# johannah/drqv2

Hardware: AMD Instinct MI355X
Metric: agent updates/sec (batch=256, 9x84x84 obs) (higher is better)
Workload: dtype f32; 1 GPU; cheetah_run batch_size=256/GPU (256 global) 9x84x84 u8 obs, A=6, feature_dim=50, hidden_dim=1024, fp32, use_tb=True; parallelism=dp1, global_batch=256

## Files before the change

drqv2_amd/_lib.py:

```python
import ctypes as C
import os

HERE = os.path.dirname(os.path.abspath(__file__))
LIB_PATH = os.path.join(HERE, "libdrqv2_hip.so")

c_float_p = C.c_void_p
c_u8_p = C.c_void_p
stream_t = C.c_void_p


class DrqStep(C.Structure):
    _fields_ = [
        ("B", C.c_int), ("global_B", C.c_int), ("C", C.c_int), ("A", C.c_int), ("F", C.c_int), ("H", C.c_int),
        ("obs", c_u8_p), ("next_obs", c_u8_p),
        ("action", c_float_p), ("reward", c_float_p), ("discount", c_float_p),
        ("shift_obs", c_float_p), ("shift_next", c_float_p),
        ("noise_critic", c_float_p), ("noise_actor", c_float_p),
        ("base_grid", c_float_p),
        ("params", c_float_p), ("grads", c_float_p), ("adam_m", c_float_p), ("adam_v", c_float_p),
        ("ws", c_float_p), ("ws_bytes", C.c_size_t),
        ("sums", c_float_p),
        ("lr", C.c_double), ("tau", C.c_double),
        ("std", C.c_float), ("clip", C.c_float),
        ("step_critic", C.c_long), ("step_enc", C.c_long), ("step_actor", C.c_long),
# ... 77 lines not shown
    "drq_tanh_bwd": (I, [P, P, P, L, P]),
    "drq_param_layout": (I, [I, I, I, I, C.POINTER(L), I]),
    "drq_step_ws_bytes": (SZ, [I, I, I, I, I]),
    "drq_step_ws_offset": (L, [I, I, I, I, I, I]),
    "drq_update_phase": (I, [C.POINTER(DrqStep), I]),
    "drq_update_phase_bc": (I, [C.POINTER(DrqStep), I, F]),
    "drq_update_phase_per": (I, [C.POINTER(DrqStep), I, P, P]),
    "drq_act_forward": (I, [C.POINTER(DrqStep), P, I, P]),
    "drq_act_ws_bytes": (SZ, [I, I, I, I, I]),
    "drq_act_batch": (I, [P, I, I, I, I, P, I, P, F, P, P, P, SZ, P]),
    "drq_publish_sums": (I, [P, P, C.c_uint, P]),
    "drq_rng_draws": (I, [C.c_uint64, C.c_uint64, I, I, I, P, P, P, P, P]),
}

WS_IDS = ["AUG", "ACT1", "ACT2", "ACT3", "FEAT", "Z_NEXT", "Z_OBS", "HA_T", "HA_C", "H_AN", "H_AO", "Q", "TQ",
          "DQ", "MU_O", "DY4", "DY3", "DY2", "DY1", "DZ_C", "DZ_A", "HA_C2", "P1", "P2", "C1", "C2"]

PHASE_ALL, PHASE_CRITIC, PHASE_ACTOR, PHASE_OPT = -1, 0, 1, 2
PHASE_ENCODE, PHASE_CRITIC_HEADS, PHASE_CONV_BACKWARD, PHASE_ACTOR_FORWARD, PHASE_ACTOR_BACKWARD = 3, 4, 5, 6, 7
PHASE_ENCODER_OPT, PHASE_ACTOR_OPT = 8, 9
PHASE_CRITIC_OPT, PHASE_ACTOR_LOSS, PHASE_POLYAK, PHASE_REDRAW = 10, 11, 12, 13

_lib = None


class DrqError(RuntimeError):
    pass


def load():
    global _lib
# ... 41 lines not shown
```

drqv2_amd/csrc/conv1aug.hip:

```cpp
#include "common.h"
#include "internal.h"
#include "wino_u.h"

namespace {

constexpr int H = 84, C = 9, PAD = 4, S = 92, HW = H * H;
constexpr int HO = 41, PO = HO * HO;
constexpr int NBAND = 5;
constexpr int MAXR = 9;
constexpr int NROWS = 2 * MAXR + 1;
constexpr int SROWS = NROWS + 2;
constexpr int XPL = 42;
constexpr int XPITCH = 2 * XPL;
constexpr int HQ = H / 4;
constexpr int CP = 5, NS = CP * 9;
constexpr int XS_FLOATS = C * NROWS * XPITCH;
constexpr int U8_DWORDS = C * SROWS * HQ;
constexpr int NDMA = (U8_DWORDS + 63) / 64;
constexpr int U8_ALLOC = NDMA * 64;
constexpr int NTHR = 256;
constexpr int NWAVE = NTHR / 64;
constexpr int MAXU = 64;
constexpr int LDS_BYTES = (XS_FLOATS + U8_ALLOC + H + 3 * MAXU) * 4;

struct Conv1AugArgs {
  const uint8_t* obs[2];
  const long* fidx[2];
  const float* shift[2];
  const float* base;
  const float* w;
  const float* bias;
  float* xaug;
  float* y;
  int n, n_store;
  unsigned y_bytes;
  int stagger;
  const float* wino_w[3];
  float* wino_u;
  int n_rider;
};

typedef float f32x2 __attribute__((ext_vector_type(2)));
typedef __bf16 bf16x8_c1 __attribute__((ext_vector_type(8)));
typedef unsigned u32x4_c1 __attribute__((ext_vector_type(4)));
typedef unsigned u32x2_c1 __attribute__((ext_vector_type(2)));

__device__ __forceinline__ unsigned pack_bf16_c1(float lo, float hi) {
  typedef __bf16 bf16x2_c1 __attribute__((ext_vector_type(2)));
  const bf16x2_c1 v = {(__bf16)lo, (__bf16)hi};
  return __builtin_bit_cast(unsigned, v);
}

__device__ __forceinline__ float div255(float v) {
  const float r = 1.0f / 255.0f;
// ... 263 lines not shown
      }
      }
      const int oy = done.r0 + oyl;
      if constexpr (YN) {
        const int yo = p0 < npix ? (((done.f * HO + oy) * HO + ox) * 16 + half * 2) * 4 : (int)0x80000000u;
#pragma unroll
        for (int g4 = 0; g4 < 4; ++g4) {
          float v[4];
#pragma unroll
          for (int e = 0; e < 4; ++e) v[e] = acc[4 * g4 + e] > 0.f ? acc[4 * g4 + e] : 0.f;
          const u32x2_c1 o = {pack_bf16_c1(v[0], v[1]), pack_bf16_c1(v[2], v[3])};
          __builtin_amdgcn_raw_buffer_store_b64(o, yrsrc, yo, g4 * 16, 0);
        }
        continue;
      }
      const int yoff = p0 < npix ? (((done.f * 32 + 4 * half) * HO + oy) * HO + ox) * 4 : (int)0x80000000u;
#pragma unroll
      for (int r = 0; r < 16; ++r) {
        const float v = acc[r] > 0.f ? acc[r] : 0.f;
        __builtin_amdgcn_raw_buffer_store_b32(__float_as_uint(v), yrsrc, yoff, ((r & 3) + 8 * (r >> 2)) * PO * 4, 0);
      }
    }
  }
}

}

int drq_conv1_aug_fwd_any(int bf_mma, const uint8_t* obs, const float* shift, const uint8_t* obs1, const float* shift1,
                          const float* base_grid, const float* w, const float* bias, float* xaug, float* y, int n,
                          int n_store, hipStream_t st, const float* const* wino_w, float* wino_u, const long* fidx0,
                          const long* fidx1) {
  if (!obs || !shift || !obs1 || !shift1 || !base_grid || !w || !bias || !y || n <= 0 || n_store < 0 || n_store > 2 * n)
    return DRQ_EARG;
  if (n_store > 0 && !xaug) return DRQ_EARG;
  if (((uintptr_t)obs & 3) || ((uintptr_t)obs1 & 3)) return DRQ_EARG;
  const size_t yb = (size_t)2 * n * 32 * PO * (bf_mma == 2 ? 2 : 4);
  if (yb >= (1ull << 31) || (bf_mma == 2 && ((uintptr_t)y & 15))) return DRQ_EARG;
  Conv1AugArgs a{};
  a.obs[0] = obs; a.obs[1] = obs1;
  a.fidx[0] = fidx0; a.fidx[1] = fidx1;
  a.shift[0] = shift; a.shift[1] = shift1;
  a.base = base_grid; a.w = w; a.bias = bias; a.xaug = xaug; a.y = y;
  a.n = n; a.n_store = n_store; a.y_bytes = (unsigned)yb; a.stagger = 1;
  if (wino_w && wino_u) {
    for (int l = 0; l < 3; ++l) a.wino_w[l] = wino_w[l];
    a.wino_u = wino_u;
    a.n_rider = 6;
  }
  static bool attr_set_dev[kMaxDevices] = {};
  bool& attr_set = attr_set_dev[drq_device()];
  if (!attr_set) {
    hipError_t e = hipFuncSetAttribute((const void*)conv1_aug_kernel<false>, hipFuncAttributeMaxDynamicSharedMemorySize,
                                       LDS_BYTES);
    if (e == hipSuccess)
      e = hipFuncSetAttribute((const void*)conv1_aug_kernel<true>, hipFuncAttributeMaxDynamicSharedMemorySize, LDS_BYTES);
    if (e == hipSuccess)
      e = hipFuncSetAttribute((const void*)conv1_aug_kernel<true, true>, hipFuncAttributeMaxDynamicSharedMemorySize,
// ... 46 lines not shown
```

drqv2_amd/csrc/conv_wino.hip:

```cpp
#include "common.h"
#include "internal.h"
#include "wino_u.h"
#include <type_traits>

namespace {

struct WinoArgs {
  const float* x;
  const float* w;
  const float* pre;
  const float* bias;
  const float* mask;
  float* y;
  int y_bs, y_cs, y_rs, y_off;
  unsigned x_bytes, y_bytes, mask_bytes;
  int nb;
  int relu;
  int wmode;
  int stagger;
};

typedef unsigned u32x4w __attribute__((ext_vector_type(4)));
typedef unsigned u32x2w __attribute__((ext_vector_type(2)));
typedef float f32x2w __attribute__((ext_vector_type(2)));

constexpr int kStagger = 0;

template <int HIN, bool MASK, bool RELU>
__global__ __launch_bounds__(256, 2) void conv3x3_wino_kernel(WinoArgs a) {
#pragma clang fp contract(off)
  constexpr int HOUT = HIN - 2;
  constexpr int TH = (HOUT + 1) / 2;
  constexpr int TT = TH * TH;
  constexpr int PLANE = HIN * HIN * 4;
  __shared__ __attribute__((aligned(16))) float U[16 * 8 * 64 * 2];

  const int tid = threadIdx.x;
  const int lane = tid & 63;
  const int wid = tid >> 6;
  const int tl = lane & 15;
  const int kk = lane >> 4;

  if (a.pre) {
    const f32x4* src = reinterpret_cast<const f32x4*>(a.pre);
    f32x4* dst = reinterpret_cast<f32x4*>(U);
// ... 10 lines not shown
  for (int h = 0; h < 2; ++h)
#pragma unroll
    for (int r = 0; r < 4; ++r) bv[h][r] = a.bias ? a.bias[16 * h + 4 * kk + r] : 0.f;
  __syncthreads();

  if (a.stagger) {
    const unsigned hwid = __builtin_amdgcn_s_getreg((4 << 0) | (0 << 6) | (31 << 11));
    if (hwid & 1u)
      for (int q = 0; q < a.stagger; ++q) __builtin_amdgcn_s_sleep(16);
  }

  const __amdgpu_buffer_rsrc_t xrs = __builtin_amdgcn_make_buffer_rsrc((void*)a.x, 0, a.x_bytes, 0x00020000);
  const __amdgpu_buffer_rsrc_t yrs = __builtin_amdgcn_make_buffer_rsrc((void*)a.y, 0, a.y_bytes, 0x00020000);
  const __amdgpu_buffer_rsrc_t mrs =
      __builtin_amdgcn_make_buffer_rsrc((void*)a.mask, 0, a.mask ? a.mask_bytes : 0, 0x00020000);
  constexpr int kDrop = (int)0x80000000u;

  const int ntile = a.nb * TT;
  const int nunit = (ntile + 15) >> 4;
  const int nwave = (int)gridDim.x * 4;
  const f32x2w* Ul = reinterpret_cast<const f32x2w*>(U) + lane;

  auto patch_voff = [&](int unit) {
    int t = unit * 16 + tl;
    t = t < ntile ? t : ntile - 1;
    const int b = t / TT, rem = t - b * TT;
    const int ty = rem / TH, tx = rem - ty * TH;
    return (((b * 32 + kk) * HIN + 2 * ty) * HIN + 2 * tx) * 4;
  };
  auto load_patch_row = [&](float (&d)[16], int voff, int c, int i) {
    const u32x4w v = __builtin_amdgcn_raw_buffer_load_b128(xrs, voff, c * (4 * PLANE) + i * (HIN * 4), 0);
// ... 49 lines not shown
    const int t = valid ? t0 : ntile - 1;
    const int b = t / TT, rem = t - b * TT;
    const int ty = rem / TH, tx = rem - ty * TH;
    const bool c1ok = 2 * tx + 1 < HOUT, r1ok = 2 * ty + 1 < HOUT;
    const int ybase = (a.y_off + b * a.y_bs + (4 * kk) * a.y_cs + (2 * ty) * a.y_rs + 2 * tx) * 4;
    const int mbase = (((b * 32 + 4 * kk) * HOUT + 2 * ty) * HOUT + 2 * tx) * 4;
    int o64[2], o32[2];
#pragma unroll
    for (int i = 0; i < 2; ++i) {
      const bool rowok = valid && (i == 0 || r1ok);
      o64[i] = (rowok && c1ok) ? ybase : kDrop;
      o32[i] = (rowok && !c1ok) ? ybase : kDrop;
    }
    f32x4 acc[16][2];
    u32x2w mk[2][4][2];
#pragma unroll
    for (int c = 0; c < 8; ++c) {
      asm volatile("" ::: "memory");
      float t[16];
#pragma unroll
      for (int j = 0; j < 4; ++j) {
        t[0 * 4 + j] = d[0 * 4 + j] - d[2 * 4 + j];
        t[1 * 4 + j] = d[1 * 4 + j] + d[2 * 4 + j];
        t[2 * 4 + j] = d[2 * 4 + j] - d[1 * 4 + j];
        t[3 * 4 + j] = d[1 * 4 + j] - d[3 * 4 + j];
      }
      __builtin_amdgcn_sched_barrier(0);
      load_A(A1, c, 1);
      __builtin_amdgcn_sched_barrier(0);
      float V[16];
// ... 17 lines not shown
          if (c == 0) {
            const f32x4 z = {0.f, 0.f, 0.f, 0.f};
            const f32x4 b0 = {bv[0][0], bv[0][1], bv[0][2], bv[0][3]}, b1 = {bv[1][0], bv[1][1], bv[1][2], bv[1][3]};
            if constexpr (HSEL != 1) acc[pos][0] = __builtin_amdgcn_mfma_f32_16x16x4f32(Ap[0], V[pos], pos == 5 ? b0 : z, 0, 0, 0);
            if constexpr (HSEL != 0) acc[pos][1] = __builtin_amdgcn_mfma_f32_16x16x4f32(Ap[1], V[pos], pos == 5 ? b1 : z, 0, 0, 0);
          } else {
            if constexpr (HSEL != 1) acc[pos][0] = __builtin_amdgcn_mfma_f32_16x16x4f32(Ap[0], V[pos], acc[pos][0], 0, 0, 0);
            if constexpr (HSEL != 0) acc[pos][1] = __builtin_amdgcn_mfma_f32_16x16x4f32(Ap[1], V[pos], acc[pos][1], 0, 0, 0);
          }
        }
      };
      half_step(A0, 0);
      __builtin_amdgcn_sched_barrier(0);
      load_A(A0, (c + 1) & 7, 0);
      if constexpr (MASK) {
        if (c == 7) {
          constexpr int h0 = HSEL == 1 ? 1 : 0;
#pragma unroll
          for (int r = 0; r < 4; ++r)
#pragma unroll
            for (int i = 0; i < 2; ++i)
              mk[h0][r][i] = __builtin_amdgcn_raw_buffer_load_b64(mrs, mbase + i * (HOUT * 4),
                                                                  (16 * h0 + r) * (HOUT * HOUT * 4), 0);
        }
      }
      __builtin_amdgcn_sched_barrier(0);
      half_step(A1, 1);
      __builtin_amdgcn_sched_barrier(0);
    }
    {
      if constexpr (MASK && HSEL == 2) {
#pragma unroll
        for (int r = 0; r < 4; ++r)
#pragma unroll
          for (int i = 0; i < 2; ++i)
            mk[1][r][i] = __builtin_amdgcn_raw_buffer_load_b64(mrs, mbase + i * (HOUT * 4), (16 + r) * (HOUT * HOUT * 4), 0);
        __builtin_amdgcn_sched_barrier(0);
      }
      const int ycs4 = a.y_cs * 4, yrs4 = a.y_rs * 4;
#pragma unroll
      for (int h = (HSEL == 1 ? 1 : 0); h < (HSEL == 0 ? 1 : 2); ++h)
#pragma unroll
        for (int r = 0; r < 4; ++r) {
          float s[2][4];
#pragma unroll
          for (int j = 0; j < 4; ++j) {
            const float m0 = acc[0 * 4 + j][h][r], m1 = acc[1 * 4 + j][h][r], m2 = acc[2 * 4 + j][h][r],
                        m3 = acc[3 * 4 + j][h][r];
            s[0][j] = (m0 + m1) + m2;
            s[1][j] = (m1 - m2) - m3;
          }
          const int co = (16 * h + r);
#pragma unroll
          for (int i = 0; i < 2; ++i) {
            float y0 = (s[i][0] + s[i][1]) + s[i][2];
            float y1 = (s[i][1] - s[i][2]) - s[i][3];
            if constexpr (RELU) {
              y0 = __builtin_fmaxf(y0, 0.f);
              y1 = __builtin_fmaxf(y1, 0.f);
            }
            if constexpr (MASK) {
              const unsigned q0 = mk[h][r][i][0], q1 = mk[h][r][i][1];
              y0 = __uint_as_float(q0) > 0.f ? y0 : 0.f;
              y1 = __uint_as_float(q1) > 0.f ? y1 : 0.f;
            }
            const int soff = co * ycs4 + i * yrs4;
            const u32x2w pk = {__float_as_uint(y0), __float_as_uint(y1)};
            __builtin_amdgcn_raw_buffer_store_b64(pk, yrs, o64[i], soff, 0);
            __builtin_amdgcn_raw_buffer_store_b32(__float_as_uint(y0), yrs, o32[i], soff, 0);
          }
        }
    }
    voff = nvoff;
  };
  for (int i = 0; i < nfull; ++i) body(std::integral_constant<int, 2>{}, item_unit(i), item_unit(i + 1 < nitem ? i + 1 : i));
  if (has_half) {
    if (half_h == 0) body(std::integral_constant<int, 0>{}, half_unit, half_unit);
    else body(std::integral_constant<int, 1>{}, half_unit, half_unit);
  }
}

template <int HIN>
int launch_wino(const WinoArgs& a0, hipStream_t st) {
  WinoArgs a = a0;
  a.stagger = kStagger;
  constexpr int HOUT = HIN - 2, TH = (HOUT + 1) / 2;
  const long nunit = ((long)a.nb * TH * TH + 15) / 16;
  long blocks = (nunit + 3) / 4;
  const long cap = 2L * drq_num_cus();
  if (blocks > cap) blocks = cap;
  if (blocks < 1) blocks = 1;
  const dim3 g((unsigned)blocks), t(256);
  if (a.mask && a.relu) hipLaunchKernelGGL((conv3x3_wino_kernel<HIN, true, true>), g, t, 0, st, a);
  else if (a.mask) hipLaunchKernelGGL((conv3x3_wino_kernel<HIN, true, false>), g, t, 0, st, a);
  else if (a.relu) hipLaunchKernelGGL((conv3x3_wino_kernel<HIN, false, true>), g, t, 0, st, a);
  else hipLaunchKernelGGL((conv3x3_wino_kernel<HIN, false, false>), g, t, 0, st, a);
  DRQ_LAUNCH_CHECK();
  return DRQ_OK;
}

}

int drq_conv3x3_fwd_wino_pre(const float* x, const float* w, const float* u_image, const float* bias, float* y, int nb,
                             int hin, int relu, long y_bs, long y_cs, long y_rs, long y_off, hipStream_t st) {
  if (!x || !w || !y || nb <= 0) return DRQ_EARG;
  const size_t xb = (size_t)nb * 32 * hin * hin * 4;
  const size_t yb = (size_t)nb * y_bs * 4;
  if (xb >= (1ull << 31) || yb >= (1ull << 31) || y_off < 0 || y_bs <= 0) return DRQ_EARG;
  WinoArgs a{x, w, u_image, bias, nullptr, y, (int)y_bs, (int)y_cs, (int)y_rs, (int)y_off, (unsigned)xb, (unsigned)yb, 0u, nb, relu, 0, 0};
  if (hin == 41) return launch_wino<41>(a, st);
  if (hin == 39) return launch_wino<39>(a, st);
  if (hin == 37) return launch_wino<37>(a, st);
  return DRQ_EARG;
}

int drq_conv3x3_dgrad_wino_pre(const float* dy_pad, const float* w, const float* u_image, const float* mask, float* dx,
                               int nb, int hout, long dx_bs, long dx_cs, long dx_rs, long dx_off, hipStream_t st) {
  if (!dy_pad || !w || !dx || nb <= 0) return DRQ_EARG;
  const int hp = hout + 4;
  const size_t xb = (size_t)nb * 32 * hp * hp * 4;
  const size_t yb = (size_t)nb * dx_bs * 4;
  const size_t mb = (size_t)nb * 32 * (hout + 2) * (hout + 2) * 4;
  if (xb >= (1ull << 31) || yb >= (1ull << 31) || dx_off < 0 || dx_bs <= 0) return DRQ_EARG;
  WinoArgs a{dy_pad, w, u_image, nullptr, mask, dx, (int)dx_bs, (int)dx_cs, (int)dx_rs, (int)dx_off, (unsigned)xb, (unsigned)yb,
             (unsigned)mb, nb, 0, 1, 0};
  if (hp == 39) return launch_wino<39>(a, st);
  if (hp == 41) return launch_wino<41>(a, st);
  if (hp == 43) return launch_wino<43>(a, st);
  return DRQ_EARG;
}

DRQ_API int drq_conv3x3_fwd_wino(const float* x, const float* w, const float* bias, float* y, int nb, int hin, int relu,
                                 long y_bs, long y_cs, long y_rs, long y_off, hipStream_t st) {
  return drq_conv3x3_fwd_wino_pre(x, w, nullptr, bias, y, nb, hin, relu, y_bs, y_cs, y_rs, y_off, st);
}

DRQ_API int drq_conv3x3_dgrad_wino(const float* dy_pad, const float* w, const float* mask, float* dx, int nb, int hout,
                                   long dx_bs, long dx_cs, long dx_rs, long dx_off, hipStream_t st) {
  return drq_conv3x3_dgrad_wino_pre(dy_pad, w, nullptr, mask, dx, nb, hout, dx_bs, dx_cs, dx_rs, dx_off, st);
}
```

drqv2_amd/csrc/internal.h:

```cpp
#pragma once
#include "common.h"

int drq_ln_tanh_fwd_multi_ex(int n, const float* const* z, int ldz, const float* const* gamma,
                             const float* const* beta, float* const* out, const int* ldo, float* const* xhat,
                             float* const* rstd, int rows, int F, const float* const* tail, const int* tail_ld,
                             int tail_n, hipStream_t st);
int drq_ln_tanh_fwd_multi_part(int n, const float* const* z, int ldz, const float* const* gamma,
                               const float* const* beta, float* const* out, const int* ldo, float* const* xhat,
                               float* const* rstd, int rows, int F, const float* const* tail, const int* tail_ld,
                               int tail_n, const float* part, const float* const* bias, int splitk, hipStream_t st);
int drq_ln_tanh_bwd_part(const float* dh0, int ld0, const float* dh1, int ld1, const float* h, int ldh,
                         const float* xhat, const float* rstd, const float* gamma, float* dz, float* dln,
                         float* dgamma, float* dbeta, int rows, int F, const float* part, int splitk, int nprob,
                         int ldp, hipStream_t st);
int drq_ln_param_grad(const float* dln, const float* xhat, float* dgamma, float* dbeta, int rows, int F,
                      hipStream_t st);
int drq_qout_bwd_td(const float* tq1, const float* tq2, const float* q1, const float* q2, const float* reward,
                    const float* discount, float inv_global_B, float* sums, const float* const* h,
                    const float* const* w, float* const* dh, float* const* dw, float* const* db, int B, int H,
                    hipStream_t st);
int drq_qout_bwd_td_w(const float* tq1, const float* tq2, const float* q1, const float* q2, const float* reward,
                      const float* discount, const float* is_weight, float inv_global_B, float* sums, float* td_abs,
                      const float* const* h, const float* const* w, float* const* dh, float* const* dw,
                      float* const* db, int B, int H, hipStream_t st);
// ... 52 lines not shown
                          long lddx, const float* const* mask, int ldmask, int Brows, int Nout, int Kin, hipStream_t st);

int drq_lnl1_fwd(int njobs, const float* const* part, const float* const* z, const float* const* bias,
                 const float* const* gamma, const float* const* beta, float* const* out, const int* ldo,
                 float* const* xhat, float* const* rstd, const float* const* tail, const int* tail_ld, const int* tail_n,
                 const int* rows, const int* nheads, const float* const* w, const float* const* b, float* const* y, int F,
                 int H, int splitk, long slab, hipStream_t st);
int drq_polout_l1_fwd(const float* p2, const float* w3, const float* b3, float* p3, int rows, int srow0, int H, int A,
                      int F, float std, float clip, int use_clip, const float* noise_hi, float* mu_hi, float* ha_hi,
                      long lda_hi, const float* noise_lo, float* mu_lo, float* ha_lo, long lda_lo, int nheads,
                      const float* const* w, const float* const* b, float* const* y, hipStream_t st);

int drq_conv1_aug_fwd_any(int bf_mma, const uint8_t* obs, const float* shift, const uint8_t* obs1, const float* shift1,
                          const float* base_grid, const float* w, const float* bias, float* xaug, float* y, int n,
                          int n_store, hipStream_t st, const float* const* wino_w, float* wino_u, const long* fidx0,
                          const long* fidx1);

int drq_conv3x3_fwd_wino_pre(const float* x, const float* w, const float* u_image, const float* bias, float* y, int nb,
                             int hin, int relu, long y_bs, long y_cs, long y_rs, long y_off, hipStream_t st);
int drq_conv3x3_dgrad_wino_pre(const float* dy_pad, const float* w, const float* u_image, const float* mask, float* dx,
                               int nb, int hout, long dx_bs, long dx_cs, long dx_rs, long dx_off, hipStream_t st);

int drq_conv3x3_fwd_bf16_lay(const void* x, const float* w, const float* bias, void* y, int nb, int hin, int relu,
                             long y_bs, long y_cs, long y_rs, long y_off, int lay, hipStream_t st);
int drq_conv3x3_dgrad_bf16_lay(const void* dy_pad, const float* w, const void* mask, void* dx, int nb, int hout,
                               long dx_bs, long dx_cs, long dx_rs, long dx_off, int lay, hipStream_t st);
int drq_conv3x3_wgrad_partial_bf16_lay(const void* x, const void* dy, int nb, int hin, long dy_bs, long dy_cs, long dy_rs,
                                       long dy_off, float* part, size_t part_bytes, int* nblocks, int lay,
                                       hipStream_t st);
int drq_conv3x3_wgrad_partial_bf16(const float* x, const float* dy, int nb, int hin, long dy_bs, long dy_cs, long dy_rs,
                                   long dy_off, float* part, size_t part_bytes, int* nblocks, hipStream_t st);

constexpr int kActMaxRows = 256;
struct ActWeights {
  const float *enc_w[4], *enc_b[4];
  const float *trunk_w, *trunk_b, *ln_g, *ln_b;
// ... 19 lines not shown
```

drqv2_amd/csrc/step.hip:

```cpp
#include "common.h"
#include "internal.h"
#include "../../include/drqv2_hip.h"

namespace {

constexpr long R = 32L * 35 * 35;
inline long al64(long x) { return (x + 63) & ~63L; }
inline long al512(long x) { return (x + 511) & ~511L; }

struct HeadOff {
  long trunk_w, trunk_b, ln_g, ln_b;
  long w[2][3], b[2][3];
};
enum { SEG_ENC, SEG_CRITIC, SEG_ACTOR, SEG_TARGET };
struct ParamLayout {
  long enc_w[4], enc_b[4];
  HeadOff critic, actor, target;
  long seg[8];
  long total;
  long flat[50];
  int nflat;
  long seg_beg(int net) const { return seg[2 * net]; }
  long seg_len(int net) const { return seg[2 * net + 1] - seg[2 * net]; }
};
// ... 47 lines not shown
}

struct WsLayout {
  long off[64];
  long total;
};
constexpr long kGemmWsFloats = 16L * 1024 * 1024;
enum {
  W_AUG = DRQ_WS_AUG, W_ACT1 = DRQ_WS_ACT1, W_ACT2 = DRQ_WS_ACT2, W_ACT3 = DRQ_WS_ACT3, W_FEAT = DRQ_WS_FEAT,
  W_Z_NEXT = DRQ_WS_Z_NEXT, W_Z_OBS = DRQ_WS_Z_OBS, W_HA_T = DRQ_WS_HA_T, W_HA_C = DRQ_WS_HA_C,
  W_H_AN = DRQ_WS_H_AN, W_H_AO = DRQ_WS_H_AO, W_Q = DRQ_WS_Q, W_TQ = DRQ_WS_TQ, W_DQ = DRQ_WS_DQ,
  W_MU_O = DRQ_WS_MU_O, W_DY4 = DRQ_WS_DY4, W_DY3 = DRQ_WS_DY3, W_DY2 = DRQ_WS_DY2, W_DY1 = DRQ_WS_DY1,
  W_DZ_C = DRQ_WS_DZ_C, W_DZ_A = DRQ_WS_DZ_A, W_HA_C2 = DRQ_WS_HA_C2,
  W_P1 = DRQ_WS_P1, W_P2 = DRQ_WS_P2,
  W_C1 = DRQ_WS_C1, W_C2 = DRQ_WS_C2,
  W_XHAT_C = DRQ_WS_NBUF_PUBLIC, W_RSTD_C, W_XHAT_A, W_RSTD_A, W_Z_C2,
  W_HROWS, W_P3, W_Z4,
  W_T1, W_T2,
  W_DC2, W_DC1, W_DHA, W_DLN, W_DPRE, W_DP2, W_DP1, W_DH_A, W_DA,
  W_GEMM_WS, W_CONV_WS,
  W_WINO_U,
  W_COUNT
};

WsLayout ws_layout(int B, int C, int A, int F, int H) {
  WsLayout w{};
  long off = 0;
  auto take = [&](int id, long n) {
    w.off[id] = off;
    off = al64(off + n);
// ... 35 lines not shown
  take(W_T2, 2L * B * H);
  take(W_C1, 2L * B * H);
  take(W_C2, 2L * B * H);
  take(W_DC2, 2L * B * H);
  take(W_DC1, 2L * B * H);
  take(W_DHA, 2L * B * (F + A));
  take(W_DLN, (long)B * F);
  take(W_DPRE, (long)B * A);
  take(W_DP2, (long)B * H);
  take(W_DP1, (long)B * H);
  take(W_DH_A, (long)B * F);
  take(W_DA, 2L * B * A);
  take(W_GEMM_WS, kGemmWsFloats);
  take(W_CONV_WS, (long)(drq_conv3x3_wgrad_ws_bytes() / sizeof(float)));
  take(W_WINO_U, 6L * 16384);
  w.total = off;
  return w;
}

#define CK(expr)                \
  do {                          \
    const int rc__ = (expr);    \
    if (rc__ != 0) return rc__; \
  } while (0)

struct Ctx {
  const DrqStep* s;
  ParamLayout P;
  WsLayout W;
  hipStream_t st;
  bool fuse_actor_loss = false;
  float bc_alpha = 0.f;
  bool bc() const { return bc_alpha > 0.f; }
  const float* a_beh() const { return ws(W_HA_C) + s->F; }
  float bc_scale() const { return 2.0f / ((float)s->global_B * (float)s->A); }
  const float* is_weight = nullptr;
  float* td_abs = nullptr;
  bool per() const { return is_weight != nullptr; }
  bool qout_loss_fits_lds() const { return ((size_t)s->B + 5 * 1024 + 16) * 4 <= 60 * 1024; }
  bool actor_loss_fused() const { return fuse_actor_loss && qout_loss_fits_lds(); }
  bool fuse_rows() const {
    return !(s->flags & DRQ_STEP_NO_ROW_FUSION) && !s->bf16 && s->A <= 32 && s->F + s->A <= 64 && s->F % 2 == 0 &&
           s->A % 2 == 0 && s->H % 256 == 0;
  }
  bool use_gemm3() const { return !(s->flags & DRQ_STEP_NO_GEMM3) && !s->bf16; }
  int stamp(int idx) const {
    if (s->timing_events && idx < s->timing_n && hipEventRecord((hipEvent_t)s->timing_events[idx], st) != hipSuccess)
      return DRQ_EARG;
    return 0;
  }
  float* ws(int id) const { return s->ws + W.off[id]; }
  float* p(long off) const { return s->params + off; }
  float* g(long off) const { return s->grads + off; }
  int bf16() const { return s->bf16 ? 1 : 0; }
  bool acts16() const { return s->bf16 && !(s->flags & DRQ_STEP_BF16_FP32_ACTS); }
  bool grads16() const { return acts16() && !(s->flags & DRQ_STEP_BF16_FP32_GRADS); }
  int adam_segment(int net, long step, int target = -1) const {
    const long o = P.seg_beg(net);
    return drq_adam_flat(p(o), g(o), s->adam_m + o, s->adam_v + o, P.seg_len(net), s->lr, step, s->gscale,
                         target >= 0 ? p(P.seg_beg(target)) : nullptr, target >= 0 ? s->tau : 0.0, st);
// ... 41 lines not shown
    if (use_gemm3() && n >= 2) {
      const int rc = drq_gemm3_wgrad_dgrad(n, dy, lddy, x, ldx, dw, db, w, ldw, dx, lddx, mask, ldmask, Brows, N, K, st);
      if (rc != DRQ_EARG) return rc;
    }
    if (!bf16()) {
      const int rc = drq_gemm2_wgrad_dgrad(n, dy, lddy, x, ldx, dw, db, w, ldw, dx, lddx, mask, ldmask, Brows, N, K, st);
      if (rc != DRQ_EARG) return rc;
    }
    const int rc = wgrad(n, dy, lddy, x, ldx, dw, db, Brows, N, K);
    if (rc != 0) return rc;
    return dgrad(n, dy, lddy, w, ldw, dx, lddx, Brows, K, N, mask, ldmask);
  }
};

int encoder_forward(const Ctx& c, const float* x, int nb, float* a1, float* a2, float* a3, float* a4,
                    bool timed = false) {
  const ParamLayout& P = c.P;
  float* outs[4] = {a1, a2, a3, a4};
  const float* in = x ? x : a1;
  for (int l = x ? 0 : 1; l < 4; ++l) {
    const int hin = kEncH[l], hout = kEncH[l + 1];
    if (timed && l == 1) CK(c.stamp(0));
    if (c.bf16() && l > 0)
      CK(drq_conv3x3_fwd_bf16_lay(in, c.p(P.enc_w[l]), c.p(P.enc_b[l]), outs[l], nb, hin, 1, 32L * hout * hout,
                                  (long)hout * hout, hout, 0, (x == nullptr && c.acts16()) ? (l < 3 ? 3 : 1) : 0, c.st));
    else if (l > 0)
      CK(drq_conv3x3_fwd_wino_pre(in, c.p(P.enc_w[l]), x ? nullptr : c.ws(W_WINO_U) + (2L * (l - 1)) * 16384,
                                  c.p(P.enc_b[l]), outs[l], nb, hin, 1, 32L * hout * hout, (long)hout * hout, hout, 0,
                                  c.st));
    else
      CK(drq_conv3x3_fwd(in, c.p(P.enc_w[l]), c.p(P.enc_b[l]), outs[l], nb, l == 0 ? c.s->C : 32, hin, l == 0 ? 2 : 1,
                         1, 32L * hout * hout, (long)hout * hout, hout, 0, c.st));
    if (timed && l == 1) CK(c.stamp(1));
    in = outs[l];
  }
  return 0;
}

int policy_forward(const Ctx& c, const float* h, int rows, float* p1, float* p2, float* p3, int sample_from = -1,
                   const float* noise = nullptr, float* a_out = nullptr, long lda_out = 0,
                   const float* noise0 = nullptr, float* mu_out0 = nullptr, float* a_out0 = nullptr, long lda_out0 = 0,
                   bool* did_rows0 = nullptr) {
  const DrqStep* s = c.s;
  const HeadOff& a = c.P.actor;
// ... 40 lines not shown
    if (l == 1) CK(c.fwd(2 * nn, hh1, H, w, b, y2, H, B, H, H, 1));
    if (l == 2) CK(drq_qout_fwd(2 * nn, hh2, w, b, qq, B, H, c.st));
  }
  return 0;
}

int phase_encode(const Ctx& c) {
  const DrqStep* s = c.s;
  const int B = s->B;
  hipStream_t st = c.st;
  float* aug = c.ws(W_AUG);
  const float* wino_w[3] = {c.p(c.P.enc_w[1]), c.p(c.P.enc_w[2]), c.p(c.P.enc_w[3])};
  CK(drq_conv1_aug_fwd_any(c.acts16() ? 2 : c.bf16(), s->obs, s->shift_obs, s->next_obs, s->shift_next, s->base_grid,
                           c.p(c.P.enc_w[0]), c.p(c.P.enc_b[0]), aug, c.ws(W_ACT1), B, s->store_aug_next ? 2 * B : B, st,
                           c.bf16() ? nullptr : wino_w, c.bf16() ? nullptr : c.ws(W_WINO_U), s->obs_index,
                           s->next_obs_index));
  CK(encoder_forward(c, nullptr, 2 * B, c.ws(W_ACT1), c.ws(W_ACT2), c.ws(W_ACT3), c.ws(W_FEAT), true));
  return 0;
}

int phase_critic_heads(const Ctx& c) {
  const DrqStep* s = c.s;
  const ParamLayout& P = c.P;
  const int B = s->B, A = s->A, F = s->F, H = s->H, FA = F + A;
  hipStream_t st = c.st;
  float* feat = c.ws(W_FEAT);
  float* feat_obs = feat;
  float* feat_next = feat + (long)B * R;
  const HeadOff &cr = P.critic, &ac = P.actor, &tg = P.target;
  const long BH = (long)B * H;

  float* z4 = c.ws(W_Z4);
// ... 113 lines not shown
                     c.g(cr.ln_g), c.g(cr.ln_b)));
    CK(drq_gemm_batched_any(0, 1, dz, F, 1, w, R, 0, dy4, 0, B, (int)R, F, nullptr, 0, mk, (int)R, nullptr, 35, 0, 0,
                            c.gemm_ws(), c.gemm_ws_bytes(), st));
  }

  return 0;
}

int phase_conv_backward(const Ctx& c) {
  const DrqStep* s = c.s;
  const ParamLayout& P = c.P;
  const int B = s->B, C = s->C;
  hipStream_t st = c.st;
  const int dyid[4] = {W_DY1, W_DY2, W_DY3, W_DY4};
  const int actid[4] = {W_AUG, W_ACT1, W_ACT2, W_ACT3};
  float* cws = c.ws(W_CONV_WS);
  const size_t quarter = drq_conv3x3_wgrad_ws_bytes() / 4;
  const float* parts[4];
  int nblk[4], cins[4];
  float *dws[4], *dbs[4];
  const bool merged = !c.bf16();
  for (int l = 3; l >= 0; --l) {
    const int hin = kEncH[l], hout = kEncH[l + 1], hp = hout + 4;
    const float* dy = c.ws(dyid[l]);
    float* part = cws + (size_t)l * (quarter / sizeof(float));
    parts[l] = part; cins[l] = l == 0 ? C : 32; dws[l] = c.g(P.enc_w[l]); dbs[l] = c.g(P.enc_b[l]);
    if (!merged) {
      if (l > 0)
        CK(drq_conv3x3_wgrad_partial_bf16_lay(c.ws(actid[l]), dy, B, hin, 32L * hp * hp, (long)hp * hp, hp, 2L * hp + 2,
                                              part, quarter, &nblk[l],
// ... 1 lines not shown
      else
        CK(drq_conv3x3_wgrad_partial(c.ws(actid[l]), dy, B, C, hin, 2, 32L * hp * hp, (long)hp * hp, hp, 2L * hp + 2,
                                     part, quarter, &nblk[l], st));
    }
    if (l >= 1) {
      const int hpi = hin + 4;
      if (l == 2) CK(c.stamp(2));
      if (c.bf16())
        CK(drq_conv3x3_dgrad_bf16_lay(dy, c.p(P.enc_w[l]), c.ws(actid[l]), c.ws(dyid[l - 1]), B, hout, 32L * hpi * hpi,
                                      (long)hpi * hpi, hpi, 2L * hpi + 2,
                                      (c.acts16() ? 4 : 0) | (c.grads16() && l < 3 ? 1 : 0) | (c.grads16() && l > 1 ? 2 : 0),
                                      st));
      else
        CK(drq_conv3x3_dgrad_wino_pre(dy, c.p(P.enc_w[l]), c.ws(W_WINO_U) + (2L * (l - 1) + 1) * 16384, c.ws(actid[l]),
                                      c.ws(dyid[l - 1]), B, hout, 32L * hpi * hpi, (long)hpi * hpi, hpi, 2L * hpi + 2,
                                      st));
      if (l == 2) CK(c.stamp(3));
    }
  }
  if (merged) {
    const float *xs[3], *dys[3];
    float* ps[3];
    long bs[3], cs[3], rs[3], off[3];
    for (int k = 0; k < 3; ++k) {
      const int l = k + 1, hp = kEncH[l + 1] + 4;
      xs[k] = c.ws(actid[l]); dys[k] = c.ws(dyid[l]); ps[k] = const_cast<float*>(parts[l]);
      bs[k] = 32L * hp * hp; cs[k] = (long)hp * hp; rs[k] = hp; off[k] = 2L * hp + 2;
    }
    int nb3[3];
    CK(c.stamp(4));
    int rc = drq_conv3x3_wgrad_partial_wino3(xs, dys, B, bs, cs, rs, off, ps, quarter, nb3, st);
// ... 317 lines not shown
```

include/drqv2_hip.h:

```cpp
#ifndef DRQV2_HIP_H
#define DRQV2_HIP_H
#include <stddef.h>
#include <stdint.h>

#ifdef __cplusplus
extern "C" {
#endif

typedef void* drq_stream_t;

#define DRQ_OK 0
#define DRQ_EARG (-1)
#define DRQ_EWS (-2)

int drq_abi_version(void);

int drq_aug_fwd(const uint8_t* obs, const float* shift_xy, const float* base_grid, float* out, int n, int c,
                int hw, int pad, int fuse_norm, drq_stream_t stream);
int drq_aug_fwd_f32(const float* x, const float* shift_xy, const float* base_grid, float* out, int n, int c,
                    int hw, int pad, drq_stream_t stream);

int drq_conv1_aug_fwd(const uint8_t* obs, const float* shift, const uint8_t* obs1, const float* shift1,
                      const float* base_grid, const float* w, const float* bias, float* xaug, float* y, int n,
                      int n_store, drq_stream_t stream);
// ... 188 lines not shown
  float gscale;
  drq_stream_t stream;
  float* sums_host;
  int store_aug_next;
  int bf16;
  void* const* timing_events;
  int timing_n;
  const int64_t* obs_index;
  const int64_t* next_obs_index;
  int flags;
} DrqStep;
#define DRQ_STEP_NO_ROW_FUSION 1
#define DRQ_STEP_NO_GEMM3 2
#define DRQ_STEP_BF16_FP32_ACTS 4
#define DRQ_STEP_BF16_FP32_GRADS 8

int drq_param_layout(int C, int A, int F, int H, long* out, int cap);
#define DRQ_PARAM_LAYOUT_LEN 59

size_t drq_step_ws_bytes(int B, int C, int A, int F, int H);
long drq_step_ws_offset(int B, int C, int A, int F, int H, int buffer_id);
enum {
  DRQ_WS_AUG = 0, DRQ_WS_ACT1, DRQ_WS_ACT2, DRQ_WS_ACT3, DRQ_WS_FEAT, DRQ_WS_Z_NEXT, DRQ_WS_Z_OBS,
  DRQ_WS_HA_T, DRQ_WS_HA_C, DRQ_WS_H_AN, DRQ_WS_H_AO, DRQ_WS_Q, DRQ_WS_TQ, DRQ_WS_DQ, DRQ_WS_MU_O,
  DRQ_WS_DY4, DRQ_WS_DY3, DRQ_WS_DY2, DRQ_WS_DY1, DRQ_WS_DZ_C, DRQ_WS_DZ_A, DRQ_WS_HA_C2,
  DRQ_WS_P1, DRQ_WS_P2,
  DRQ_WS_C1, DRQ_WS_C2,
  DRQ_WS_NBUF_PUBLIC
};

enum {
  DRQ_PHASE_ALL = -1, DRQ_PHASE_CRITIC = 0, DRQ_PHASE_ACTOR = 1, DRQ_PHASE_OPT = 2,
  DRQ_PHASE_ENCODE = 3, DRQ_PHASE_CRITIC_HEADS = 4, DRQ_PHASE_CONV_BACKWARD = 5, DRQ_PHASE_ACTOR_FORWARD = 6,
  DRQ_PHASE_ACTOR_BACKWARD = 7, DRQ_PHASE_ENCODER_OPT = 8, DRQ_PHASE_ACTOR_OPT = 9,
  DRQ_PHASE_CRITIC_OPT = 10, DRQ_PHASE_ACTOR_LOSS = 11, DRQ_PHASE_POLYAK = 12, DRQ_PHASE_REDRAW = 13
};
int drq_update_phase(const DrqStep* s, int phase);
int drq_update_phase_bc(const DrqStep* s, int phase, float bc_alpha);
int drq_update_phase_per(const DrqStep* s, int phase, const float* is_weight, float* td_abs);

int drq_publish_sums(const float* sums, float* sums_host, unsigned seq, drq_stream_t stream);

// ... 11 lines not shown
```

Baseline: 977.8 updates/s.

## Pack ReLU masks into bit words during forward and use them in conv dgrad

```diff
diff --git a/drqv2_amd/_lib.py b/drqv2_amd/_lib.py
--- a/drqv2_amd/_lib.py
+++ b/drqv2_amd/_lib.py
@@ -115,7 +115,8 @@
 }
 
 WS_IDS = ["AUG", "ACT1", "ACT2", "ACT3", "FEAT", "Z_NEXT", "Z_OBS", "HA_T", "HA_C", "H_AN", "H_AO", "Q", "TQ",
-          "DQ", "MU_O", "DY4", "DY3", "DY2", "DY1", "DZ_C", "DZ_A", "HA_C2", "P1", "P2", "C1", "C2"]
+          "DQ", "MU_O", "DY4", "DY3", "DY2", "DY1", "DZ_C", "DZ_A", "HA_C2", "P1", "P2", "C1", "C2",
+          "MASK1", "MASK2", "MASK3"]
 
 PHASE_ALL, PHASE_CRITIC, PHASE_ACTOR, PHASE_OPT = -1, 0, 1, 2
 PHASE_ENCODE, PHASE_CRITIC_HEADS, PHASE_CONV_BACKWARD, PHASE_ACTOR_FORWARD, PHASE_ACTOR_BACKWARD = 3, 4, 5, 6, 7
diff --git a/drqv2_amd/csrc/conv1aug.hip b/drqv2_amd/csrc/conv1aug.hip
--- a/drqv2_amd/csrc/conv1aug.hip
+++ b/drqv2_amd/csrc/conv1aug.hip
@@ -38,6 +38,7 @@
   const float* wino_w[3];
   float* wino_u;
   int n_rider;
+  unsigned* mbits;
 };
 
 typedef float f32x2 __attribute__((ext_vector_type(2)));
@@ -331,6 +332,17 @@
         }
         continue;
       }
+      if constexpr (!BF) {
+        if (a.mbits && done.f < a.n) {
+          const __amdgpu_buffer_rsrc_t mrsrc =
+              __builtin_amdgcn_make_buffer_rsrc((void*)a.mbits, 0, (unsigned)a.n * (PO * 4), 0x00020000);
+          unsigned bits = 0;
+#pragma unroll
+          for (int r = 0; r < 16; ++r) bits |= (acc[r] > 0.f ? 1u : 0u) << r;
+          const int moff = p0 < npix ? (((done.f * HO + oy) * HO + ox) * 2 + half) * 2 : (int)0x80000000u;
+          __builtin_amdgcn_raw_buffer_store_b16((unsigned short)bits, mrsrc, moff, 0, 0);
+        }
+      }
       const int yoff = p0 < npix ? (((done.f * 32 + 4 * half) * HO + oy) * HO + ox) * 4 : (int)0x80000000u;
 #pragma unroll
       for (int r = 0; r < 16; ++r) {
@@ -346,7 +358,8 @@
 int drq_conv1_aug_fwd_any(int bf_mma, const uint8_t* obs, const float* shift, const uint8_t* obs1, const float* shift1,
                           const float* base_grid, const float* w, const float* bias, float* xaug, float* y, int n,
                           int n_store, hipStream_t st, const float* const* wino_w, float* wino_u, const long* fidx0,
-                          const long* fidx1) {
+                          const long* fidx1, unsigned* mask_pixels) {
+  if (mask_pixels && (bf_mma || (size_t)n * PO * 4 >= (1ull << 31))) return DRQ_EARG;
   if (!obs || !shift || !obs1 || !shift1 || !base_grid || !w || !bias || !y || n <= 0 || n_store < 0 || n_store > 2 * n)
     return DRQ_EARG;
   if (n_store > 0 && !xaug) return DRQ_EARG;
@@ -358,6 +371,7 @@
   a.fidx[0] = fidx0; a.fidx[1] = fidx1;
   a.shift[0] = shift; a.shift[1] = shift1;
   a.base = base_grid; a.w = w; a.bias = bias; a.xaug = xaug; a.y = y;
+  a.mbits = mask_pixels;
   a.n = n; a.n_store = n_store; a.y_bytes = (unsigned)yb; a.stagger = 1;
   if (wino_w && wino_u) {
     for (int l = 0; l < 3; ++l) a.wino_w[l] = wino_w[l];
diff --git a/drqv2_amd/csrc/conv_wino.hip b/drqv2_amd/csrc/conv_wino.hip
--- a/drqv2_amd/csrc/conv_wino.hip
+++ b/drqv2_amd/csrc/conv_wino.hip
@@ -18,6 +18,10 @@
   int relu;
   int wmode;
   int stagger;
+  unsigned* words;
+  unsigned words_bytes;
+  int n_word_frames;
+  int words_kind;
 };
 
 typedef unsigned u32x4w __attribute__((ext_vector_type(4)));
@@ -26,9 +30,10 @@
 
 constexpr int kStagger = 0;
 
-template <int HIN, bool MASK, bool RELU>
+template <int HIN, bool MASK, bool RELU, int FMASK = 1>
 __global__ __launch_bounds__(256, 2) void conv3x3_wino_kernel(WinoArgs a) {
 #pragma clang fp contract(off)
+  constexpr int WORDS = FMASK ? 0 : (HIN == 43 ? 2 : 1);
   constexpr int HOUT = HIN - 2;
   constexpr int TH = (HOUT + 1) / 2;
   constexpr int TT = TH * TH;
@@ -69,7 +74,10 @@
   const __amdgpu_buffer_rsrc_t yrs = __builtin_amdgcn_make_buffer_rsrc((void*)a.y, 0, a.y_bytes, 0x00020000);
   const __amdgpu_buffer_rsrc_t mrs =
       __builtin_amdgcn_make_buffer_rsrc((void*)a.mask, 0, a.mask ? a.mask_bytes : 0, 0x00020000);
+  const __amdgpu_buffer_rsrc_t wrs =
+      __builtin_amdgcn_make_buffer_rsrc((void*)a.words, 0, WORDS ? a.words_bytes : 0, 0x00020000);
   constexpr int kDrop = (int)0x80000000u;
+  const int wsh = 16 * (kk & 1) + 4 * (kk >> 1);
 
   const int ntile = a.nb * TT;
   const int nunit = (ntile + 15) >> 4;
@@ -149,6 +157,11 @@
     }
     f32x4 acc[16][2];
     u32x2w mk[2][4][2];
+    unsigned mw = 0;
+    u32x2w mp[2] = {};
+    const int woff = (unit * 64 + lane) * 4;
+    const int wst = (valid && b < a.n_word_frames) ? woff : kDrop;
+    const int poff = ((b * HOUT + 2 * ty) * HOUT + 2 * tx) * 4;
 #pragma unroll
     for (int c = 0; c < 8; ++c) {
       asm volatile("" ::: "memory");
@@ -196,7 +209,12 @@
       __builtin_amdgcn_sched_barrier(0);
       load_A(A0, (c + 1) & 7, 0);
       if constexpr (MASK) {
-        if (c == 7) {
+        if (c == 7 && WORDS == 1) {
+          mw = __builtin_amdgcn_raw_buffer_load_b32(wrs, woff, 0, 0);
+        } else if (c == 7 && WORDS == 2) {
+#pragma unroll
+          for (int i = 0; i < 2; ++i) mp[i] = __builtin_amdgcn_raw_buffer_load_b64(wrs, poff + i * (HOUT * 4), 0, 0);
+        } else if (c == 7) {
           constexpr int h0 = HSEL == 1 ? 1 : 0;
 #pragma unroll
           for (int r = 0; r < 4; ++r)
@@ -211,7 +229,7 @@
       __builtin_amdgcn_sched_barrier(0);
     }
     {
-      if constexpr (MASK && HSEL == 2) {
+      if constexpr (MASK && HSEL == 2 && WORDS == 0) {
 #pragma unroll
         for (int r = 0; r < 4; ++r)
 #pragma unroll
@@ -220,6 +238,11 @@
         __builtin_amdgcn_sched_barrier(0);
       }
       const int ycs4 = a.y_cs * 4, yrs4 = a.y_rs * 4;
+      if constexpr (WORDS == 2) {
+        mp[0] = mp[0] >> (unsigned)wsh;
+        mp[1] = mp[1] >> (unsigned)wsh;
+      }
+      unsigned wbits[2] = {0u, 0u};
 #pragma unroll
       for (int h = (HSEL == 1 ? 1 : 0); h < (HSEL == 0 ? 1 : 2); ++h)
 #pragma unroll
@@ -241,7 +264,22 @@
               y0 = __builtin_fmaxf(y0, 0.f);
               y1 = __builtin_fmaxf(y1, 0.f);
             }
-            if constexpr (MASK) {
+            if constexpr (RELU && !MASK && WORDS == 1) {
+              const int s0 = (int)__float_as_uint(y0), s1 = (int)__float_as_uint(y1);
+              wbits[h] |= (unsigned)(s0 > 0 ? 1 : 0) << (4 * r + 2 * i);
+              wbits[h] |= (unsigned)(s1 > 0 ? 1 : 0) << (4 * r + 2 * i + 1);
+            }
+            if constexpr (MASK && WORDS == 1) {
+              const int k = 16 * h + 4 * r + 2 * i;
+              const unsigned k0 = (unsigned)(-(int)((mw >> k) & 1u)), k1 = (unsigned)(-(int)((mw >> (k + 1)) & 1u));
+              y0 = __uint_as_float(__float_as_uint(y0) & k0);
+              y1 = __uint_as_float(__float_as_uint(y1) & k1);
+            } else if constexpr (MASK && WORDS == 2) {
+              const int k = 8 * h + r;
+              const unsigned k0 = (unsigned)(-(int)((mp[i][0] >> k) & 1u)), k1 = (unsigned)(-(int)((mp[i][1] >> k) & 1u));
+              y0 = __uint_as_float(__float_as_uint(y0) & k0);
+              y1 = __uint_as_float(__float_as_uint(y1) & k1);
+            } else if constexpr (MASK) {
               const unsigned q0 = mk[h][r][i][0], q1 = mk[h][r][i][1];
               y0 = __uint_as_float(q0) > 0.f ? y0 : 0.f;
               y1 = __uint_as_float(q1) > 0.f ? y1 : 0.f;
@@ -252,6 +290,12 @@
             __builtin_amdgcn_raw_buffer_store_b32(__float_as_uint(y0), yrs, o32[i], soff, 0);
           }
         }
+      if constexpr (RELU && !MASK && WORDS == 1) {
+        if constexpr (HSEL == 2)
+          __builtin_amdgcn_raw_buffer_store_b32(wbits[0] | (wbits[1] << 16), wrs, wst, 0, 0);
+        else
+          __builtin_amdgcn_raw_buffer_store_b16((unsigned short)wbits[HSEL], wrs, wst, 2 * HSEL, 0);
+      }
     }
     voff = nvoff;
   };
@@ -273,6 +317,28 @@
   if (blocks > cap) blocks = cap;
   if (blocks < 1) blocks = 1;
   const dim3 g((unsigned)blocks), t(256);
+  if (a.words_kind) {
+    if constexpr (HIN == 39 || HIN == 41) {
+      if (a.words_kind == 1 && a.relu && !a.mask) {
+        hipLaunchKernelGGL((conv3x3_wino_kernel<HIN, false, true, 0>), g, t, 0, st, a);
+        DRQ_LAUNCH_CHECK();
+        return DRQ_OK;
+      }
+      if (a.words_kind == 1 && !a.relu) {
+        hipLaunchKernelGGL((conv3x3_wino_kernel<HIN, true, false, 0>), g, t, 0, st, a);
+        DRQ_LAUNCH_CHECK();
+        return DRQ_OK;
+      }
+    }
+    if constexpr (HIN == 43) {
+      if (a.words_kind == 2 && !a.relu) {
+        hipLaunchKernelGGL((conv3x3_wino_kernel<HIN, true, false, 0>), g, t, 0, st, a);
+        DRQ_LAUNCH_CHECK();
+        return DRQ_OK;
+      }
+    }
+    return DRQ_EARG;
+  }
   if (a.mask && a.relu) hipLaunchKernelGGL((conv3x3_wino_kernel<HIN, true, true>), g, t, 0, st, a);
   else if (a.mask) hipLaunchKernelGGL((conv3x3_wino_kernel<HIN, true, false>), g, t, 0, st, a);
   else if (a.relu) hipLaunchKernelGGL((conv3x3_wino_kernel<HIN, false, true>), g, t, 0, st, a);
@@ -284,12 +350,20 @@
 }
 
 int drq_conv3x3_fwd_wino_pre(const float* x, const float* w, const float* u_image, const float* bias, float* y, int nb,
-                             int hin, int relu, long y_bs, long y_cs, long y_rs, long y_off, hipStream_t st) {
+                             int hin, int relu, long y_bs, long y_cs, long y_rs, long y_off, hipStream_t st,
+                             unsigned* mask_words, int n_word_frames) {
   if (!x || !w || !y || nb <= 0) return DRQ_EARG;
+  if (mask_words && (!relu || n_word_frames < 0 || n_word_frames > nb || (hin != 41 && hin != 39))) return DRQ_EARG;
   const size_t xb = (size_t)nb * 32 * hin * hin * 4;
   const size_t yb = (size_t)nb * y_bs * 4;
   if (xb >= (1ull << 31) || yb >= (1ull << 31) || y_off < 0 || y_bs <= 0) return DRQ_EARG;
   WinoArgs a{x, w, u_image, bias, nullptr, y, (int)y_bs, (int)y_cs, (int)y_rs, (int)y_off, (unsigned)xb, (unsigned)yb, 0u, nb, relu, 0, 0};
+  if (mask_words) {
+    a.words = mask_words;
+    a.words_bytes = (unsigned)(drq_mask_tile_words(n_word_frames, hin - 2) * 4);
+    a.n_word_frames = n_word_frames;
+    a.words_kind = 1;
+  }
   if (hin == 41) return launch_wino<41>(a, st);
   if (hin == 39) return launch_wino<39>(a, st);
   if (hin == 37) return launch_wino<37>(a, st);
@@ -297,8 +371,10 @@
 }
 
 int drq_conv3x3_dgrad_wino_pre(const float* dy_pad, const float* w, const float* u_image, const float* mask, float* dx,
-                               int nb, int hout, long dx_bs, long dx_cs, long dx_rs, long dx_off, hipStream_t st) {
+                               int nb, int hout, long dx_bs, long dx_cs, long dx_rs, long dx_off, hipStream_t st,
+                               const unsigned* mask_words) {
   if (!dy_pad || !w || !dx || nb <= 0) return DRQ_EARG;
+  if (mask_words && hout != 35 && hout != 37 && hout != 39) return DRQ_EARG;
   const int hp = hout + 4;
   const size_t xb = (size_t)nb * 32 * hp * hp * 4;
   const size_t yb = (size_t)nb * dx_bs * 4;
@@ -306,6 +382,12 @@
   if (xb >= (1ull << 31) || yb >= (1ull << 31) || dx_off < 0 || dx_bs <= 0) return DRQ_EARG;
   WinoArgs a{dy_pad, w, u_image, nullptr, mask, dx, (int)dx_bs, (int)dx_cs, (int)dx_rs, (int)dx_off, (unsigned)xb, (unsigned)yb,
              (unsigned)mb, nb, 0, 1, 0};
+  if (mask_words) {
+    a.mask = nullptr;
+    a.words = const_cast<unsigned*>(mask_words);
+    a.words_kind = hp == 43 ? 2 : 1;
+    a.words_bytes = (unsigned)((hp == 43 ? drq_mask_pixel_words(nb) : drq_mask_tile_words(nb, hout + 2)) * 4);
+  }
   if (hp == 39) return launch_wino<39>(a, st);
   if (hp == 41) return launch_wino<41>(a, st);
   if (hp == 43) return launch_wino<43>(a, st);
@@ -314,10 +396,10 @@
 
 DRQ_API int drq_conv3x3_fwd_wino(const float* x, const float* w, const float* bias, float* y, int nb, int hin, int relu,
                                  long y_bs, long y_cs, long y_rs, long y_off, hipStream_t st) {
-  return drq_conv3x3_fwd_wino_pre(x, w, nullptr, bias, y, nb, hin, relu, y_bs, y_cs, y_rs, y_off, st);
+  return drq_conv3x3_fwd_wino_pre(x, w, nullptr, bias, y, nb, hin, relu, y_bs, y_cs, y_rs, y_off, st, nullptr, 0);
 }
 
 DRQ_API int drq_conv3x3_dgrad_wino(const float* dy_pad, const float* w, const float* mask, float* dx, int nb, int hout,
                                    long dx_bs, long dx_cs, long dx_rs, long dx_off, hipStream_t st) {
-  return drq_conv3x3_dgrad_wino_pre(dy_pad, w, nullptr, mask, dx, nb, hout, dx_bs, dx_cs, dx_rs, dx_off, st);
-}
+  return drq_conv3x3_dgrad_wino_pre(dy_pad, w, nullptr, mask, dx, nb, hout, dx_bs, dx_cs, dx_rs, dx_off, st, nullptr);
+}
diff --git a/drqv2_amd/csrc/internal.h b/drqv2_amd/csrc/internal.h
--- a/drqv2_amd/csrc/internal.h
+++ b/drqv2_amd/csrc/internal.h
@@ -90,12 +90,20 @@
 int drq_conv1_aug_fwd_any(int bf_mma, const uint8_t* obs, const float* shift, const uint8_t* obs1, const float* shift1,
                           const float* base_grid, const float* w, const float* bias, float* xaug, float* y, int n,
                           int n_store, hipStream_t st, const float* const* wino_w, float* wino_u, const long* fidx0,
-                          const long* fidx1);
+                          const long* fidx1, unsigned* mask_pixels = nullptr);
+
+inline long drq_mask_tile_words(int frames, int hout) {
+  const long th = (hout + 1) / 2;
+  return (frames * th * th + 15) / 16 * 64;
+}
+inline long drq_mask_pixel_words(int frames) { return (long)frames * 41 * 41; }
 
 int drq_conv3x3_fwd_wino_pre(const float* x, const float* w, const float* u_image, const float* bias, float* y, int nb,
-                             int hin, int relu, long y_bs, long y_cs, long y_rs, long y_off, hipStream_t st);
+                             int hin, int relu, long y_bs, long y_cs, long y_rs, long y_off, hipStream_t st,
+                             unsigned* mask_words, int n_word_frames);
 int drq_conv3x3_dgrad_wino_pre(const float* dy_pad, const float* w, const float* u_image, const float* mask, float* dx,
-                               int nb, int hout, long dx_bs, long dx_cs, long dx_rs, long dx_off, hipStream_t st);
+                               int nb, int hout, long dx_bs, long dx_cs, long dx_rs, long dx_off, hipStream_t st,
+                               const unsigned* mask_words);
 
 int drq_conv3x3_fwd_bf16_lay(const void* x, const float* w, const float* bias, void* y, int nb, int hin, int relu,
                              long y_bs, long y_cs, long y_rs, long y_off, int lay, hipStream_t st);
diff --git a/drqv2_amd/csrc/step.hip b/drqv2_amd/csrc/step.hip
--- a/drqv2_amd/csrc/step.hip
+++ b/drqv2_amd/csrc/step.hip
@@ -85,6 +85,7 @@
   W_DZ_C = DRQ_WS_DZ_C, W_DZ_A = DRQ_WS_DZ_A, W_HA_C2 = DRQ_WS_HA_C2,
   W_P1 = DRQ_WS_P1, W_P2 = DRQ_WS_P2,
   W_C1 = DRQ_WS_C1, W_C2 = DRQ_WS_C2,
+  W_MASK1 = DRQ_WS_MASK1, W_MASK2 = DRQ_WS_MASK2, W_MASK3 = DRQ_WS_MASK3,
   W_XHAT_C = DRQ_WS_NBUF_PUBLIC, W_RSTD_C, W_XHAT_A, W_RSTD_A, W_Z_C2,
   W_HROWS, W_P3, W_Z4,
   W_T1, W_T2,
@@ -150,6 +151,9 @@
   take(W_GEMM_WS, kGemmWsFloats);
   take(W_CONV_WS, (long)(drq_conv3x3_wgrad_ws_bytes() / sizeof(float)));
   take(W_WINO_U, 6L * 16384);
+  take(W_MASK1, drq_mask_pixel_words(B));
+  take(W_MASK2, drq_mask_tile_words(B, 39));
+  take(W_MASK3, drq_mask_tile_words(B, 37));
   w.total = off;
   return w;
 }
@@ -180,6 +184,8 @@
            s->A % 2 == 0 && s->H % 256 == 0;
   }
   bool use_gemm3() const { return !(s->flags & DRQ_STEP_NO_GEMM3) && !s->bf16; }
+  bool mask_words() const { return !(s->flags & DRQ_STEP_FP32_MASKS) && !s->bf16; }
+  unsigned* mask_ws(int id) const { return reinterpret_cast<unsigned*>(ws(id)); }
   int stamp(int idx) const {
     if (s->timing_events && idx < s->timing_n && hipEventRecord((hipEvent_t)s->timing_events[idx], st) != hipSuccess)
       return DRQ_EARG;
@@ -251,7 +257,7 @@
 };
 
 int encoder_forward(const Ctx& c, const float* x, int nb, float* a1, float* a2, float* a3, float* a4,
-                    bool timed = false) {
+                    bool timed = false, int n_word_frames = 0) {
   const ParamLayout& P = c.P;
   float* outs[4] = {a1, a2, a3, a4};
   const float* in = x ? x : a1;
@@ -264,7 +270,8 @@
     else if (l > 0)
       CK(drq_conv3x3_fwd_wino_pre(in, c.p(P.enc_w[l]), x ? nullptr : c.ws(W_WINO_U) + (2L * (l - 1)) * 16384,
                                   c.p(P.enc_b[l]), outs[l], nb, hin, 1, 32L * hout * hout, (long)hout * hout, hout, 0,
-                                  c.st));
+                                  c.st, (n_word_frames > 0 && l < 3) ? c.mask_ws(l == 1 ? W_MASK2 : W_MASK3) : nullptr,
+                                  n_word_frames));
     else
       CK(drq_conv3x3_fwd(in, c.p(P.enc_w[l]), c.p(P.enc_b[l]), outs[l], nb, l == 0 ? c.s->C : 32, hin, l == 0 ? 2 : 1,
                          1, 32L * hout * hout, (long)hout * hout, hout, 0, c.st));
@@ -335,8 +342,9 @@
   CK(drq_conv1_aug_fwd_any(c.acts16() ? 2 : c.bf16(), s->obs, s->shift_obs, s->next_obs, s->shift_next, s->base_grid,
                            c.p(c.P.enc_w[0]), c.p(c.P.enc_b[0]), aug, c.ws(W_ACT1), B, s->store_aug_next ? 2 * B : B, st,
                            c.bf16() ? nullptr : wino_w, c.bf16() ? nullptr : c.ws(W_WINO_U), s->obs_index,
-                           s->next_obs_index));
-  CK(encoder_forward(c, nullptr, 2 * B, c.ws(W_ACT1), c.ws(W_ACT2), c.ws(W_ACT3), c.ws(W_FEAT), true));
+                           s->next_obs_index, c.mask_words() ? c.mask_ws(W_MASK1) : nullptr));
+  CK(encoder_forward(c, nullptr, 2 * B, c.ws(W_ACT1), c.ws(W_ACT2), c.ws(W_ACT3), c.ws(W_FEAT), true,
+                     c.mask_words() ? B : 0));
   return 0;
 }
 
@@ -480,6 +488,7 @@
   hipStream_t st = c.st;
   const int dyid[4] = {W_DY1, W_DY2, W_DY3, W_DY4};
   const int actid[4] = {W_AUG, W_ACT1, W_ACT2, W_ACT3};
+  const int maskid[4] = {-1, W_MASK1, W_MASK2, W_MASK3};
   float* cws = c.ws(W_CONV_WS);
   const size_t quarter = drq_conv3x3_wgrad_ws_bytes() / 4;
   const float* parts[4];
@@ -511,7 +520,7 @@
       else
         CK(drq_conv3x3_dgrad_wino_pre(dy, c.p(P.enc_w[l]), c.ws(W_WINO_U) + (2L * (l - 1) + 1) * 16384, c.ws(actid[l]),
                                       c.ws(dyid[l - 1]), B, hout, 32L * hpi * hpi, (long)hpi * hpi, hpi, 2L * hpi + 2,
-                                      st));
+                                      st, c.mask_words() ? c.mask_ws(maskid[l]) : nullptr));
       if (l == 2) CK(c.stamp(3));
     }
   }
diff --git a/include/drqv2_hip.h b/include/drqv2_hip.h
--- a/include/drqv2_hip.h
+++ b/include/drqv2_hip.h
@@ -226,6 +226,7 @@
 #define DRQ_STEP_NO_GEMM3 2
 #define DRQ_STEP_BF16_FP32_ACTS 4
 #define DRQ_STEP_BF16_FP32_GRADS 8
+#define DRQ_STEP_FP32_MASKS 16
 
 int drq_param_layout(int C, int A, int F, int H, long* out, int cap);
 #define DRQ_PARAM_LAYOUT_LEN 59
@@ -238,6 +239,7 @@
   DRQ_WS_DY4, DRQ_WS_DY3, DRQ_WS_DY2, DRQ_WS_DY1, DRQ_WS_DZ_C, DRQ_WS_DZ_A, DRQ_WS_HA_C2,
   DRQ_WS_P1, DRQ_WS_P2,
   DRQ_WS_C1, DRQ_WS_C2,
+  DRQ_WS_MASK1, DRQ_WS_MASK2, DRQ_WS_MASK3,
   DRQ_WS_NBUF_PUBLIC
 };
 
```

Result: no change. 977.1 updates/s (-0.1%).
